# MrTornado24/FENeRF

Hardware: NVIDIA H100
Metric: rendered faces/sec at 128px x 24 samples/ray (higher is better)
Workload: dtype f16 operands / f32 accumulate (wgmma) + f32 refinement

## Files before the change

### fenerf_b200/csrc/layout.h

```cpp
#pragma once
#include <stddef.h>
#include <stdint.h>
#include "../../include/fenerf_b200.h"

#define FN_H 256
#define FN_MAX_HIDDEN 15
#define FN_KCHUNK 64
#define FN_IMG_BYTES (256 * FN_KCHUNK * 2)
#define FN_SLOT_POS 0
#define FN_SLOT_DIR 16
#define FN_SLOT_FEAT 32
#define FN_SPLIT_SCALES (FN_MAX_HIDDEN + 3)

#define FN_HEAD_IMG_BYTES(rows) ((size_t)(FN_H / FN_KCHUNK) * (rows) * FN_KCHUNK * 2)
constexpr int FN_FEAT = 64;
constexpr int FN_FEAT_SIGMA_ROW = 0;

struct FnHead {
    size_t w;
    size_t img;
    int32_t n_out, w_rows, img_rows;
};

struct FnLayout {
// ... 138 lines not shown
        L->head_img_s = take(FN_HEAD_IMG_BYTES(32));
        L->head_img_lo = take(FN_HEAD_IMG_BYTES(32));
        L->rgb_img_s = take(FN_HEAD_IMG_BYTES(8));
        L->rgb_img_lo = take(FN_HEAD_IMG_BYTES(8));
        L->split_scale = take(2 * FN_SPLIT_SCALES * 4);
    }
    L->total = off;
    return 0;
}

#if defined(__CUDACC__)
__host__ __device__
#endif
static inline uint32_t fn_sw128_offset(uint32_t row, uint32_t k) {
    return (row >> 3) * 1024u + (row & 7u) * 128u + ((((k >> 3) ^ (row & 7u)) & 7u) << 4) + (k & 7u) * 2u;
}

#if defined(__CUDACC__)
__host__ __device__
#endif
static inline uint32_t fn_hidden_img_offset(uint32_t n, uint32_t k) {
    return (n >> 7) * 65536u + (k / FN_KCHUNK) * 16384u + fn_sw128_offset(n & 127u, k % FN_KCHUNK);
}
```

### fenerf_b200/csrc/pack.cu

```cuda
#include "common.cuh"

namespace fn {

namespace {

__device__ __forceinline__ __half f16_hi(float w) { return __float2half_rn(w); }
__device__ __forceinline__ __half f16_lo(float w) { return __float2half_rn(w - __half2float(__float2half_rn(w))); }

__global__ void pack_first_kernel(const float* __restrict__ w, int g, const float* __restrict__ b,
                                  float* __restrict__ wt, float* __restrict__ bo, unsigned char* __restrict__ img,
                                  unsigned char* __restrict__ img_lo) {
    int n = blockIdx.x * blockDim.x + threadIdx.x;
    if (n >= FN_H) return;
    const int in_dim = g + 3;
    bo[n] = b[n];
    for (int k = 0; k < FN_KCHUNK; ++k) *reinterpret_cast<__half*>(img + fn_sw128_offset(n, k)) = __float2half_rn(0.f);
    for (int k = 0; k < 3; ++k) {
        float v = w[n * in_dim + g + k];
        wt[k * FN_H + n] = v;
        *reinterpret_cast<__half*>(img + fn_sw128_offset(n, FN_SLOT_POS + k)) = f16_hi(v);
        *reinterpret_cast<__half*>(img + fn_sw128_offset(n, FN_SLOT_POS + 3 + k)) = f16_hi(v);
        *reinterpret_cast<__half*>(img + fn_sw128_offset(n, FN_SLOT_POS + 6 + k)) = f16_lo(v);
    }
    if (img_lo)
        for (int k = 0; k < FN_KCHUNK; ++k) *reinterpret_cast<__half*>(img_lo + fn_sw128_offset(n, k)) = __float2half_rn(0.f);
    for (int c = 0; c < g; ++c) {
        const float v = w[n * in_dim + c];
        wt[(3 + c) * FN_H + n] = v;
        *reinterpret_cast<__half*>(img + fn_sw128_offset(n, FN_SLOT_FEAT + c)) = f16_hi(v);
        *reinterpret_cast<__half*>(img_lo + fn_sw128_offset(n, FN_SLOT_FEAT + c)) = f16_lo(v);
    }
}

__global__ void pack_hidden_kernel(const float* __restrict__ w, const float* __restrict__ b, int in_dim, int x_off,
                                   int kx, int kx_pad, float* __restrict__ wt, float* __restrict__ bo,
                                   unsigned char* __restrict__ img) {
    __shared__ float tile[32][33];
    int k0 = blockIdx.x * 32, n0 = blockIdx.y * 32;
    int k_total = FN_H + kx_pad;
    for (int i = threadIdx.y; i < 32; i += blockDim.y) {
        int n = n0 + i, k = k0 + threadIdx.x;
        float v = 0.f;
        if (k < FN_H) v = w[(size_t)n * in_dim + x_off + k];
        else if (k - FN_H < kx) v = w[(size_t)n * in_dim + (k - FN_H)];
        tile[i][threadIdx.x] = v;
    }
    __syncthreads();
    for (int i = threadIdx.y; i < 32; i += blockDim.y) {
        int k = k0 + i, n = n0 + threadIdx.x;
        if (k < k_total) wt[(size_t)k * FN_H + n] = tile[threadIdx.x][i];
    }
    for (int i = threadIdx.y; i < 32; i += blockDim.y) {
        int n = n0 + i, k = k0 + threadIdx.x;
        if (k < FN_H)
            *reinterpret_cast<__half*>(img + fn_hidden_img_offset(n, k)) = __float2half_rn(tile[i][threadIdx.x]);
    }
    if (blockIdx.x == 0 && threadIdx.y == 0) bo[n0 + threadIdx.x] = b[n0 + threadIdx.x];
}

__global__ void pack_color0_ximg_kernel(const float* __restrict__ w, int in_dim, int g, unsigned char* __restrict__ img) {
    int n = blockIdx.x * blockDim.x + threadIdx.x;
    if (n >= FN_H) return;
    for (int k = 0; k < FN_KCHUNK; ++k) *reinterpret_cast<__half*>(img + fn_sw128_offset(n, k)) = __float2half_rn(0.f);
    for (int k = 0; k < 3; ++k) {
        float v = w[(size_t)n * in_dim + k];
        *reinterpret_cast<__half*>(img + fn_sw128_offset(n, FN_SLOT_DIR + k)) = f16_hi(v);
        *reinterpret_cast<__half*>(img + fn_sw128_offset(n, FN_SLOT_DIR + 3 + k)) = f16_hi(v);
        *reinterpret_cast<__half*>(img + fn_sw128_offset(n, FN_SLOT_DIR + 6 + k)) = f16_lo(v);
    }
    for (int c = 0; c < g; ++c)
        *reinterpret_cast<__half*>(img + fn_sw128_offset(n, FN_SLOT_FEAT + c)) = __float2half_rn(w[(size_t)n * in_dim + 3 + c]);
}

__global__ void pack_wo_dir_color0_kernel(const float* __restrict__ w, int g, int kx_pad, const float* __restrict__ b,
                                          float* __restrict__ wt, float* __restrict__ bo, unsigned char* __restrict__ img,
                                          unsigned char* __restrict__ ximg) {
    const int n = blockIdx.x;
    const size_t in_dim = (size_t)g + FN_H;
    for (int k = threadIdx.x; k < FN_H + kx_pad; k += blockDim.x) {
        float v = 0.f;
        if (k < FN_H) {
            v = w[n * in_dim + g + k];
            *reinterpret_cast<__half*>(img + fn_hidden_img_offset(n, k)) = __float2half_rn(v);
        } else if (k - FN_H >= 3 && k - FN_H < 3 + g) {
            v = w[n * in_dim + (k - FN_H - 3)];
        }
        wt[(size_t)k * FN_H + n] = v;
    }
    for (int k = threadIdx.x; k < FN_KCHUNK; k += blockDim.x) {
        const int c = k - FN_SLOT_FEAT;
        const float v = c >= 0 && c < g ? w[n * in_dim + c] : 0.f;
        *reinterpret_cast<__half*>(ximg + fn_sw128_offset(n, k)) = __float2half_rn(v);
    }
    if (threadIdx.x == 0) bo[n] = b[n];
}

__global__ void label_step1_kernel(const float* __restrict__ w3, const float* __restrict__ b3,
                                   const float* __restrict__ w2, const float* __restrict__ b2,
                                   double* __restrict__ u ) {
    int i = blockIdx.x, j = threadIdx.x;
    if (!w2) {
        u[i * (FN_H + 1) + j] = (double)w3[i * FN_H + j];
        if (j == 0) u[i * (FN_H + 1) + FN_H] = (double)b3[i];
        return;
    }
    double acc = 0.0;
// ... 343 lines not shown
        FN_REQUIRE(w && b, "weight/bias of hidden layer %d missing", l);
        if (L.bridge && is_c0) {
            FN_REQUIRE(!L.bridge_res || (bridge->pre_w && bridge->pre_b), "color_layer_pre missing");
            pack_bridge_color0_kernel<<<1, 256, 0, st>>>(w, L.bridge_res ? 3 + FN_H : 6, b,
                                                         L.bridge_res ? bridge->pre_w : nullptr,
                                                         L.bridge_res ? bridge->pre_b : nullptr,
                                                         (float*)(packed + L.hid_w32[l]), (float*)(packed + L.hid_b[l]),
                                                         packed + L.color0_ximg);
            FN_LAUNCH_OK("pack_bridge_color0_kernel");
            continue;
        }
        if (L.wo_dir && is_c0) {
            pack_wo_dir_color0_kernel<<<FN_H, 256, 0, st>>>(w, L.grid_channels, L.kx_pad, b, (float*)(packed + L.hid_w32[l]),
                                                            (float*)(packed + L.hid_b[l]), packed + L.hid_img[l],
                                                            packed + L.color0_ximg);
            FN_LAUNCH_OK("pack_wo_dir_color0_kernel");
            continue;
        }
        int in_dim = is_c0 ? L.kx + FN_H : FN_H;
        int x_off = is_c0 ? L.kx : 0;
        int kx = is_c0 ? L.kx : 0, kx_pad = is_c0 ? L.kx_pad : 0;
        dim3 grid((FN_H + kx_pad + 31) / 32, FN_H / 32), block(32, 8);
        pack_hidden_kernel<<<grid, block, 0, st>>>(w, b, in_dim, x_off, kx, kx_pad, (float*)(packed + L.hid_w32[l]),
                                                   (float*)(packed + L.hid_b[l]), packed + L.hid_img[l]);
        FN_LAUNCH_OK("pack_hidden_kernel");
        if (is_c0) {
            pack_color0_ximg_kernel<<<1, 256, 0, st>>>(w, in_dim, L.kx - 3, packed + L.color0_ximg);
            FN_LAUNCH_OK("pack_color0_ximg_kernel");
        }
    }
    FN_REQUIRE((L.bridge_res || (p->sigma_w && p->sigma_b)) && p->rgb_w && p->rgb_b, "sigma/rgb head parameters missing");
    pack_linear_head_kernel<<<1, 256, 0, st>>>(p->rgb_w, p->rgb_b, L.rgb, packed);
    FN_LAUNCH_OK("pack_linear_head_kernel");
    if (L.label_film) {
        pack_linear_head_kernel<<<1, 256, 0, st>>>(p->label_w[2], p->label_b[2], L.label, packed);
        FN_LAUNCH_OK("pack_linear_head_kernel");
    } else if (L.trunk_labels > 0) {
        for (int i = 0; i < 3; i += 2) FN_REQUIRE(p->label_w[i] && p->label_b[i], "label layer %d missing", i);
        FN_REQUIRE((p->label_w[1] == nullptr) == (p->label_b[1] == nullptr), "label layer 1: weight and bias must both be given or both be NULL");
        double* u = reinterpret_cast<double*>(packed + L.label_scratch);
        label_step1_kernel<<<L.label_dim, FN_H, 0, st>>>(p->label_w[2], p->label_b[2], p->label_w[1], p->label_b[1], u);
        FN_LAUNCH_OK("label_step1_kernel");
        label_step2_kernel<<<L.label_dim, FN_H, 0, st>>>(u, p->label_w[0], p->label_b[0], L.label_dim,
                                                         (float*)(packed + L.label_w));
        FN_LAUNCH_OK("label_step2_kernel");
        label_step3_kernel<<<1, 256, 0, st>>>((float*)(packed + L.label_w), L.label_dim);
        FN_LAUNCH_OK("label_step3_kernel");
// ... 42 lines not shown
```

### fenerf_b200/csrc/siren_fast.cu

```cuda
#include "siren_fast.cuh"

namespace fn {

int siren_fast_label_launch(const void* args, int blocks, cudaStream_t st);
int siren_fast_hd_launch(const void* args, int blocks, bool label_film, cudaStream_t st);
int siren_fast_grid_launch(const void* args, int blocks, cudaStream_t st);
int siren_fast_bridge_launch(const void* args, int blocks, cudaStream_t st);
int siren_fast_debug_launch(const void* args, int blocks, bool label_film, bool feature_head, int variant, cudaStream_t st);

namespace {

std::atomic<int> g_variant{0};
unsigned long long* g_trace = nullptr;
int g_trace_ctas = 0;

bool build_loads(const FnLayout& L, FastArgs& A, bool sigma_only) {
    A.n_loads = 0;
    auto push = [&](size_t src, uint32_t bytes) {
        if (A.n_loads < MAX_LOADS) A.loads[A.n_loads] = Load{(uint32_t)src, bytes};
        ++A.n_loads;
    };
    push(L.first_img, 2 * CHUNK);
    if (L.grid_trunk) push(L.first_img_lo, 2 * CHUNK);
    for (int l = 0; l < L.n_hidden; ++l) {
        if (l == L.trunk_hidden) {
            push(L.head_img, 4 * HEAD_CHUNK);
            if (sigma_only) return A.n_loads <= MAX_LOADS;
        }
        if (L.bridge && l == L.color0) {
            push(L.color0_ximg, 2 * CHUNK);
            continue;
        }
        push(L.hid_img[l], 2 * CHUNK);
        push(L.hid_img[l] + 2 * CHUNK, 2 * CHUNK);
        if (l == L.label_layer) push(L.label.img, (uint32_t)FN_HEAD_IMG_BYTES(L.label.img_rows));
        if (l == L.color0) push(L.color0_ximg, 2 * CHUNK);
        push(L.hid_img[l] + 4 * CHUNK, 2 * CHUNK);
        push(L.hid_img[l] + 6 * CHUNK, 2 * CHUNK);
    }
    push(L.rgb.img, (uint32_t)FN_HEAD_IMG_BYTES(L.rgb.img_rows));
    return A.n_loads <= MAX_LOADS;
}

}

int siren_fast_debug_variant(int variant, unsigned long long* trace, int trace_ctas) {
    FN_REQUIRE(variant >= 0 && variant <= 3, "unknown point-network variant %d", variant);
    FN_REQUIRE(variant < 2 || (trace && trace_ctas >= 1), "a timeline variant needs its trace buffer");
    g_trace = trace;
    g_trace_ctas = trace_ctas;
    g_variant.store(variant);
    return 0;
}

int siren_points_fast(const FnLayout& L, const unsigned char* packed, const float* points, const float* dirs, const float* film,
                      int batch, long long ppb, int dir_group, int lock_dirs, float* out, int sigma_only, cudaStream_t st,
                      float* sigma_out) {
    static_assert(sizeof(FastArgs) <= 4000, "kernel parameter block too large");
    static_assert(SMEM_TOTAL <= 232448, "one CTA per SM: 227 KB of shared memory");
    static_assert(FN_HEAD_IMG_BYTES(FN_FEAT) == SLOT_BYTES, "a feature-head image is one ring slot");
    const bool trunk_only = L.feature_head && sigma_only;
// ... 41 lines not shown
```

### fenerf_b200/csrc/siren_fast.cuh

```cuda
#pragma once
#include "common.cuh"
#include "siren_common.cuh"
#include "sm90.cuh"

namespace fn {

namespace {

using namespace sm90;

constexpr int TILE = 64;
constexpr int NTHREADS = 384;
constexpr int PROD_WARP = 8;
constexpr int RING = 6;
constexpr uint32_t SLOT_BYTES = 32768;
constexpr int XSTRIDE = 72;
constexpr uint32_t SMEM_X = RING * SLOT_BYTES;
constexpr int FRING = 2;
constexpr uint32_t FILM_BYTES = 2 * FN_H * 4;
constexpr uint32_t SMEM_FILM = SMEM_X + 2 * TILE * XSTRIDE * 2;
constexpr uint32_t SMEM_BAR = SMEM_FILM + 2 * FRING * FILM_BYTES;
constexpr uint32_t SMEM_TOTAL = SMEM_BAR + 16 * RING + 16 + 16 * 2 * FRING;
constexpr uint32_t SMEM_XLO = SMEM_TOTAL;
constexpr int XLO_STRIDE = 32;
// ... 46 lines not shown
    uint32_t bytes;
};

template <int kMaxLoads>
struct FastArgsT {
    Load loads[kMaxLoads];
    int n_loads;
    FnLayout L;
    const unsigned char* packed;
    const float* points;
    const float* dirs;
    const float* film;
    float* out;
    float* sigma_out;
    long long ppb, tiles_per_batch, n_tiles;
    int dir_group, lock_dirs;
    int sigma_only;
    unsigned long long* trace;
    int trace_ctas;
};
using FastArgs = FastArgsT<MAX_LOADS>;
using SplitArgs = FastArgsT<MAX_LOADS_SPLIT>;

__device__ __forceinline__ void wg_bar(int wg) { asm volatile("bar.sync %0, 128;" ::"r"(1 + wg) : "memory"); }

template <bool kLabelFilm, bool kFeatureHead = false, int kSoftSin = kSoftSinEvery, bool kTrace = false,
          bool kGridTrunk = false, bool kBridge = false, bool kSplit = false>
__global__ void __launch_bounds__(NTHREADS, 1)
    siren_fast_kernel(const __grid_constant__ FastArgsT<kSplit ? MAX_LOADS_SPLIT : MAX_LOADS> a) {
    constexpr int RING = kSplit ? RING_SPLIT : fn::RING;
    constexpr uint32_t SMEM_X = kSplit ? SPLIT_SMEM_X : fn::SMEM_X;
    constexpr uint32_t SMEM_FILM = kSplit ? SPLIT_SMEM_FILM : fn::SMEM_FILM;
    constexpr uint32_t SMEM_BAR = kSplit ? SPLIT_SMEM_BAR : fn::SMEM_BAR;
    constexpr uint32_t SMEM_XLO = kSplit ? SPLIT_SMEM_XLO : fn::SMEM_XLO;
    extern __shared__ __align__(1024) unsigned char smem[];
    const uint32_t sbase = smem_u32(smem);
    const int warp = threadIdx.x >> 5, lane = threadIdx.x & 31;
    const uint32_t bar_full = sbase + SMEM_BAR, bar_empty = bar_full + 8 * RING, bar_turn = bar_empty + 8 * RING;
    const uint32_t bar_ffull = bar_turn + 16, bar_fempty = bar_ffull + 8 * 2 * FRING;
    unsigned long long* tbuf = nullptr;
    uint32_t tn = 0;
    if constexpr (kTrace)
        if (lane == 0 && (int)blockIdx.x < a.trace_ctas) tbuf = a.trace + ((size_t)blockIdx.x * TRACE_WARPS + warp) * TRACE_CAP;
    auto trace = [&](int kind, int group = 0) {
        if constexpr (kTrace)
            if (tbuf && tn < TRACE_CAP)
// ... 60 lines not shown
                }
            }
        }
        return;
    }

    asm volatile("setmaxnreg.inc.sync.aligned.u32 232;\n" ::: "memory");
    const int wg = warp >> 2, q = lane & 3;
    const int tid = threadIdx.x & 127;
    const int r0 = (warp & 3) * 16 + (lane >> 2);
    const FnLayout& L = a.L;
    const int C = L.out_dim;
    const float* sigma_w = reinterpret_cast<const float*>(a.packed + L.sigma_w);
    const float* label_w = reinterpret_cast<const float*>(a.packed + L.label_w);
    const int trunk_labels = (kLabelFilm || kFeatureHead) ? 0 : L.trunk_labels;
    const int sigma_row = kFeatureHead ? FN_FEAT_SIGMA_ROW : L.sigma_row;
    const int rgb_rows = kFeatureHead ? FN_FEAT : L.rgb.w_rows;
    const int label_rows = kFeatureHead ? FN_FEAT : L.label.w_rows;
    __half* xs = reinterpret_cast<__half*>(smem + SMEM_X) + wg * TILE * XSTRIDE;
    uint32_t it = 0;
    auto acquire = [&](uint32_t& slot) -> uint32_t {
        slot = it % RING;
        trace(TR_ACQ_WAIT);
        mbar_wait(bar_full + 8 * slot, (it / RING) & 1u);
        trace(TR_ACQ_DONE);
        ++it;
        return sbase + slot * SLOT_BYTES;
    };
    auto release = [&](uint32_t slot) {
        __syncwarp();
        if (lane == 0) mbar_arrive(bar_empty + 8 * slot);
    };
    uint32_t turns = 0;
    uint32_t fit = 0;
    auto film_acquire = [&]() -> const float4* {
        const uint32_t e = wg * FRING + fit % FRING;
        trace(TR_FILM_WAIT);
        mbar_wait(bar_ffull + 8 * e, (fit / FRING) & 1u);
        trace(TR_FILM_DONE);
        return reinterpret_cast<const float4*>(smem + SMEM_FILM + e * FILM_BYTES);
    };
    auto film_release = [&]() {
        const uint32_t e = wg * FRING + fit % FRING;
        ++fit;
        __syncwarp();
        if (lane == 0) mbar_arrive(bar_fempty + 8 * e);
    };
    auto turn_begin = [&]() {
        trace(TR_TURN_WAIT);
        mbar_wait(bar_turn + 8 * wg, (turns & 1u) ^ (wg == 0 ? 1u : 0u));
        trace(TR_TURN_DONE);
    };
    auto turn_end = [&](int group) {
        trace(TR_COMMIT, group);
        ++turns;
        __syncwarp();
        if (lane == 0) mbar_arrive(bar_turn + 8 * (wg ^ 1));
    };
    auto xfrag = [&](int s, uint32_t (&f)[4]) {
        const __half* p = xs + r0 * XSTRIDE + 16 * s + 2 * q;
        f[0] = *reinterpret_cast<const uint32_t*>(p);
        f[1] = *reinterpret_cast<const uint32_t*>(p + 8 * XSTRIDE);
        f[2] = *reinterpret_cast<const uint32_t*>(p + 8);
        f[3] = *reinterpret_cast<const uint32_t*>(p + 8 * XSTRIDE + 8);
    };

    for (long long pair = blockIdx.x; pair < n_pairs; pair += gridDim.x) {
        const long long tile = pair * 2 + wg;
        const bool tile_ok = tile < a.n_tiles;
        const long long b = tile_ok ? tile / a.tiles_per_batch : 0;
        const long long p0 = tile_ok ? (tile % a.tiles_per_batch) * TILE : a.ppb;
        trace(TR_PAIR);

// ... 31 lines not shown
                if (valid && (kGridTrunk || (L.grid_channels > 0 && !a.sigma_only))) {
                    float feat[32];
                    grid_features32(reinterpret_cast<const float*>(a.packed + L.grid), L.grid_res, pos[0], pos[1], pos[2], feat);
#pragma unroll
                    for (int i = 0; i < 32; ++i) split_f16(feat[i], slots[FN_SLOT_FEAT + i], lo[i]);
                }
                __half* xlo = reinterpret_cast<__half*>(smem + SMEM_XLO) + (wg * TILE + tid) * XLO_STRIDE;
#pragma unroll
                for (int i = 0; i < 4; ++i) reinterpret_cast<uint4*>(xlo)[i] = reinterpret_cast<const uint4*>(lo)[i];
            } else if (L.grid_channels > 0 && valid && !a.sigma_only) {
                float feat[32];
                grid_features32_h(reinterpret_cast<const __half*>(a.packed + L.grid16), L.grid_res, pos[0], pos[1], pos[2], feat);
#pragma unroll
                for (int i = 0; i < 32; ++i) slots[FN_SLOT_FEAT + i] = __float2half_rn(feat[i]);
            }
#pragma unroll
            for (int i = 0; i < 8; ++i)
                reinterpret_cast<uint4*>(xs + tid * XSTRIDE)[i] = reinterpret_cast<const uint4*>(slots)[i];
        }
        wg_bar(wg);

        uint32_t act[16][4];
        uint32_t nxt[8][4];
        float d[64];
        auto film_epi = [&](const float4* fs, int h, uint32_t (&dst)[8][4]) {
#pragma unroll
            for (int j = 0; j < 16; ++j) {
                const float4 e = fs[64 * h + 4 * j + q];
                const bool soft = kSoftSin > 0 && j % (kSoftSin > 0 ? kSoftSin : 1) == kSoftSin - 1;
                auto sn = [soft](float x) { return soft ? soft_sinf(x) : __sinf(x); };
                dst[j >> 1][(j & 1) * 2] = pack_half2(sn(fmaf(e.x, d[4 * j], e.z)), sn(fmaf(e.y, d[4 * j + 1], e.w)));
                dst[j >> 1][(j & 1) * 2 + 1] = pack_half2(sn(fmaf(e.x, d[4 * j + 2], e.z)), sn(fmaf(e.y, d[4 * j + 3], e.w)));
            }
            trace(TR_EPI_DONE);
        };
        auto act_hi = [&]() -> uint32_t (&)[8][4] { return *reinterpret_cast<uint32_t (*)[8][4]>(&act[8]); };
        auto film_epi_split = [&](const float4* fs, int h, uint32_t (&dst)[8][4], uint32_t (&lo)[8][4]) {
#pragma unroll
            for (int j = 0; j < 16; ++j) {
                const float4 e = fs[64 * h + 4 * j + q];
#pragma unroll
                for (int rr = 0; rr < 2; ++rr) {
                    const float s0 = soft_sinf(fmaf(e.x, d[4 * j + 2 * rr], e.z));
                    const float s1 = soft_sinf(fmaf(e.y, d[4 * j + 2 * rr + 1], e.w));
                    const __half2 hi = __floats2half2_rn(s0, s1);
                    const float2 hf = __half22float2(hi);
                    dst[j >> 1][(j & 1) * 2 + rr] = *reinterpret_cast<const uint32_t*>(&hi);
// ... 21 lines not shown
            wg_bar(wg);
        };
        uint32_t lo0[8][4], lo1[8][4];

        {
            uint32_t xf[4], slot, slot_lo = 0, w_lo = 0;
            uint32_t xg[2][4], xl[2][4];
            const float4* fs = nullptr;
            xfrag(0, xf);
            if constexpr (kGridTrunk) {
                const __half* xlo = reinterpret_cast<const __half*>(smem + SMEM_XLO) + wg * TILE * XLO_STRIDE;
#pragma unroll
                for (int s = 0; s < 2; ++s) {
                    xfrag(2 + s, xg[s]);
                    const __half* p = xlo + r0 * XLO_STRIDE + 16 * s + 2 * q;
                    xl[s][0] = *reinterpret_cast<const uint32_t*>(p);
                    xl[s][1] = *reinterpret_cast<const uint32_t*>(p + 8 * XLO_STRIDE);
                    xl[s][2] = *reinterpret_cast<const uint32_t*>(p + 8);
                    xl[s][3] = *reinterpret_cast<const uint32_t*>(p + 8 * XLO_STRIDE + 8);
                }
            }
            const uint32_t w = acquire(slot);
            if constexpr (kGridTrunk) w_lo = acquire(slot_lo);
#pragma unroll
            for (int h = 0; h < 2; ++h) {
                turn_begin();
                wg_fence();
                mma_rs_n128(d, xf, desc_kmajor(w + h * CHUNK), 0u);
                if constexpr (kGridTrunk)
#pragma unroll
                    for (int s = 0; s < 2; ++s) {
                        mma_rs_n128(d, xg[s], desc_kmajor(w + h * CHUNK + 32 * (2 + s)), 1u);
                        mma_rs_n128(d, xl[s], desc_kmajor(w + h * CHUNK + 32 * (2 + s)), 1u);
                        mma_rs_n128(d, xg[s], desc_kmajor(w_lo + h * CHUNK + 32 * (2 + s)), 1u);
                    }
                wg_commit();
                turn_end(TG_FIRST);
                wg_wait<0>();
                trace(TR_MMA_DONE);
                fence_regs(d);
                fence_regs(xf);
                if constexpr (kGridTrunk) { fence_regs(xg); fence_regs(xl); }
                if (h == 0) fs = film_acquire();
                if constexpr (kSplit) {
                    if (h == 0) film_epi_split(fs, 0, nxt, lo0);
                    else film_epi_split(fs, 1, act_hi(), lo1);
                } else {
                    if (h == 0) film_epi(fs, 0, nxt);
                    else film_epi(fs, 1, act_hi());
                }
            }
            release(slot);
            if constexpr (kGridTrunk) release(slot_lo);
            film_release();
            if constexpr (kSplit) alo_store(lo0, lo1);
#pragma unroll
            for (int s = 0; s < 8; ++s)
#pragma unroll
                for (int i = 0; i < 4; ++i) act[s][i] = nxt[s][i];
        }

        bool stop = false;
        for (int l = 0; l < L.n_hidden && !stop; ++l) {
            if (l == L.trunk_hidden) {
                float dh[16];
                uint32_t slot, slot_lo = 0, w_lo = 0;
                const uint32_t w = acquire(slot);
                if constexpr (kSplit) w_lo = acquire(slot_lo);
                turn_begin();
                wg_fence();
#pragma unroll
                for (int c = 0; c < 4; ++c)
#pragma unroll
                    for (int k = 0; k < 4; ++k) mma_rs_n32(dh, act[4 * c + k], desc_kmajor(w + c * HEAD_CHUNK + 32 * k), (c | k) ? 1u : 0u);
                if constexpr (kSplit)
#pragma unroll
                    for (int c = 0; c < 4; ++c)
#pragma unroll
                        for (int k = 0; k < 4; ++k) {
                            mma_ss_n32(dh, alo_desc(4 * c + k), desc_kmajor(w + c * HEAD_CHUNK + 32 * k), 1u);
                            mma_rs_n32(dh, act[4 * c + k], desc_kmajor(w_lo + c * HEAD_CHUNK + 32 * k), 1u);
                        }
// ... 64 lines not shown
                        }
                    }
                    if (!a.sigma_only) wg_bar(wg);
                }
                if (a.sigma_only) { stop = true; break; }
                if constexpr (kLabelFilm) {
                    constexpr int kLabN = kFeatureHead ? FN_FEAT : 32;
                    constexpr uint32_t kLabChunk = kFeatureHead ? FEAT_CHUNK : HEAD_CHUNK;
                    float dl[kLabN / 2];
                    uint32_t slot_h = 0, w_h = 0;
                    const float4* fs = nullptr;
#pragma unroll
                    for (int h = 0; h < 2; ++h) {
                        uint32_t sl[2];
                        turn_begin();
                        wg_fence();
#pragma unroll
                        for (int sb = 0; sb < 2; ++sb) {
                            const uint32_t w = acquire(sl[sb]);
#pragma unroll
                            for (int c = 0; c < 2; ++c)
#pragma unroll
                                for (int k = 0; k < 4; ++k)
                                    mma_rs_n128(d, act[8 * sb + 4 * c + k], desc_kmajor(w + c * CHUNK + 32 * k), (sb | c | k) ? 1u : 0u);
                        }
                        wg_commit();
                        turn_end(TG_LABEL_LAYER);
                        wg_wait<0>();
                        trace(TR_MMA_DONE);
                        fence_regs(d);
                        fence_regs(act);
                        release(sl[0]);
                        release(sl[1]);
                        if (h == 0) fs = film_acquire();
                        film_epi(fs, h, nxt);
                        if (h == 0) w_h = acquire(slot_h);
                        turn_begin();
                        wg_fence();
#pragma unroll
                        for (int s = 0; s < 8; ++s) {
                            const int g = 8 * h + s;
                            const uint64_t desc = desc_kmajor(w_h + (g >> 2) * kLabChunk + 32 * (g & 3));
                            if constexpr (kFeatureHead) mma_rs_n64(dl, nxt[s], desc, (h | s) ? 1u : 0u);
                            else mma_rs_n32(dl, nxt[s], desc, (h | s) ? 1u : 0u);
                        }
                        wg_commit();
                        turn_end(TG_LABEL_HEAD);
                        wg_wait<0>();
                        trace(TR_MMA_DONE);
                        fence_regs(dl);
                        fence_regs(nxt);
                    }
                    release(slot_h);
// ... 69 lines not shown
                                mma_rs_n128(d, xl[s], desc_kmajor(w_x + off), 1u);
                                mma_rs_n128(d, xf[1 + s], desc_kmajor(w_xl + off), 1u);
                            }
                        wg_commit();
                        turn_end(TG_COLOR0);
                        wg_wait<0>();
                        trace(TR_MMA_DONE);
                        fence_regs(d);
                        fence_regs(xf);
                        fence_regs(xl);
                        release(slot_x);
                        if (grid) release(slot_xl);
                    }
                    if (h == 0) fs = film_acquire();
                    if (h == 0) film_epi_split(fs, 0, nxt, lo0);
                    else film_epi_split(fs, 1, act_hi(), lo1);
                }
                film_release();
                alo_store(lo0, lo1);
#pragma unroll
                for (int s = 0; s < 8; ++s)
#pragma unroll
                    for (int i = 0; i < 4; ++i) act[s][i] = nxt[s][i];
                continue;
            }
            const bool narrow = kBridge && c0;
            const int nx = kBridge ? 2 : !kGridTrunk && L.grid_channels > 0 ? 3 : 1;
            uint32_t xf[3][4];
            if (c0)
#pragma unroll
                for (int s = 0; s < 3; ++s) xfrag(1 + s, xf[s]);
            uint32_t slot_x = 0, w_x = 0;
            const float4* fs = nullptr;
#pragma unroll
            for (int h = 0; h < 2; ++h) {
                uint32_t sl[2] = {0u, 0u};
                if (narrow && h == 0) w_x = acquire(slot_x);
                turn_begin();
                wg_fence();
                if (!narrow)
#pragma unroll
                    for (int sb = 0; sb < 2; ++sb) {
                        const uint32_t w = acquire(sl[sb]);
#pragma unroll
                        for (int c = 0; c < 2; ++c)
#pragma unroll
                            for (int k = 0; k < 4; ++k)
                                mma_rs_n128(d, act[8 * sb + 4 * c + k], desc_kmajor(w + c * CHUNK + 32 * k), (sb | c | k) ? 1u : 0u);
                    }
                if (c0) {
                    if (h == 0 && !narrow) w_x = acquire(slot_x);
#pragma unroll
                    for (int s = 0; s < 3; ++s)
                        if (s < nx) mma_rs_n128(d, xf[s], desc_kmajor(w_x + h * CHUNK + 32 * (1 + s)), (narrow && s == 0) ? 0u : 1u);
                }
                wg_commit();
                turn_end(c0 ? TG_COLOR0 : TG_HIDDEN);
                wg_wait<0>();
                trace(TR_MMA_DONE);
                fence_regs(d);
                fence_regs(act);
                fence_regs(xf);
                if (!narrow) {
                    release(sl[0]);
                    release(sl[1]);
                }
                if (c0 && h == 1) release(slot_x);
                if (h == 0) fs = film_acquire();
                if (h == 0) film_epi(fs, 0, nxt);
                else film_epi(fs, 1, act_hi());
            }
            film_release();
#pragma unroll
            for (int s = 0; s < 8; ++s)
#pragma unroll
                for (int i = 0; i < 4; ++i) act[s][i] = nxt[s][i];
        }
        if (stop) continue;

        if constexpr (kFeatureHead) {
            float dr[32];
            uint32_t slot;
            const uint32_t w = acquire(slot);
            turn_begin();
            wg_fence();
#pragma unroll
            for (int c = 0; c < 4; ++c)
#pragma unroll
                for (int k = 0; k < 4; ++k) mma_rs_n64(dr, act[4 * c + k], desc_kmajor(w + c * FEAT_CHUNK + 32 * k), (c | k) ? 1u : 0u);
            wg_commit();
            turn_end(TG_OUT_HEAD);
            wg_wait<0>();
            trace(TR_MMA_DONE);
            fence_regs(dr);
            fence_regs(act);
            release(slot);
            const float* rgb_b = reinterpret_cast<const float*>(a.packed + L.rgb.w) + rgb_rows * FN_H;
#pragma unroll
            for (int rr = 0; rr < 2; ++rr) {
// ... 69 lines not shown
```

### fenerf_b200/csrc/sm90.cuh

```cuda
#pragma once
#include "common.cuh"

namespace fn {
namespace sm90 {

__device__ __forceinline__ uint32_t smem_u32(const void* p) { return (uint32_t)__cvta_generic_to_shared(p); }

__device__ __forceinline__ void mbar_init(uint32_t bar, uint32_t count) {
    asm volatile("mbarrier.init.shared::cta.b64 [%0], %1;" ::"r"(bar), "r"(count));
}
__device__ __forceinline__ void fence_barrier_init() { asm volatile("fence.mbarrier_init.release.cluster;" ::: "memory"); }
__device__ __forceinline__ void mbar_arrive(uint32_t bar) {
    asm volatile("{\n\t.reg .b64 st;\n\tmbarrier.arrive.shared::cta.b64 st, [%0];\n\t}" ::"r"(bar) : "memory");
}
__device__ __forceinline__ void mbar_arrive_expect_tx(uint32_t bar, uint32_t bytes) {
    asm volatile("{\n\t.reg .b64 st;\n\tmbarrier.arrive.expect_tx.shared::cta.b64 st, [%0], %1;\n\t}" ::"r"(bar), "r"(bytes)
                 : "memory");
}
__device__ __forceinline__ void mbar_wait(uint32_t bar, uint32_t parity) {
    const long long t0 = clock64();
    for (;;) {
        uint32_t done;
        asm volatile("{\n\t.reg .pred p;\n\tmbarrier.try_wait.parity.shared::cta.b64 p, [%1], %2;\n\tselp.u32 %0, 1, 0, p;\n\t}"
                     : "=r"(done) : "r"(bar), "r"(parity) : "memory");
// ... 33 lines not shown
}
template <int M, int N>
__device__ __forceinline__ void fence_regs(uint32_t (&r)[M][N]) {
#pragma unroll
    for (int i = 0; i < M; ++i) fence_regs(r[i]);
}

__device__ __forceinline__ uint64_t desc_sw128(uint32_t smem_addr, uint32_t lbo, uint32_t sbo) {
    return (uint64_t)((smem_addr >> 4) & 0x3FFF) | ((uint64_t)((lbo >> 4) & 0x3FFF) << 16) |
           ((uint64_t)((sbo >> 4) & 0x3FFF) << 32) | (1ull << 62);
}
__device__ __forceinline__ uint64_t desc_kmajor(uint32_t smem_addr) { return desc_sw128(smem_addr, 16, 1024); }

__device__ __forceinline__ uint32_t pack_half2(float a, float b) {
    __half2 h = __floats2half2_rn(a, b);
    return *reinterpret_cast<uint32_t*>(&h);
}
__device__ __forceinline__ void split_f16(float v, __half& hi, __half& lo) {
    hi = __float2half_rn(v);
    lo = __float2half_rn(v - __half2float(hi));
}


__device__ __forceinline__ void mma_rs_n128(float (&d)[64], const uint32_t (&a)[4], uint64_t b_desc, uint32_t acc) {
    asm volatile(
        "{\n\t.reg .pred p;\n\tsetp.ne.b32 p, %69, 0;\n\t"
        "wgmma.mma_async.sync.aligned.m64n128k16.f32.f16.f16 {%0, %1, %2, %3, %4, %5, %6, %7, %8, %9, %10, %11, %12, %13, %14, %15, %16, %17, %18, %19, %20, %21, %22, %23, %24, %25, %26, %27, %28, %29, %30, %31, %32, %33, %34, %35, %36, %37, %38, %39, %40, %41, %42, %43, %44, %45, %46, %47, %48, %49, %50, %51, %52, %53, %54, %55, %56, %57, %58, %59, %60, %61, %62, %63}, {%64, %65, %66, %67}, %68, p, 1, 1, 0;\n\t}"
        : "+f"(d[0]), "+f"(d[1]), "+f"(d[2]), "+f"(d[3]), "+f"(d[4]), "+f"(d[5]), "+f"(d[6]), "+f"(d[7]), "+f"(d[8]), "+f"(d[9]), "+f"(d[10]), "+f"(d[11]), "+f"(d[12]), "+f"(d[13]), "+f"(d[14]), "+f"(d[15]), "+f"(d[16]), "+f"(d[17]), "+f"(d[18]), "+f"(d[19]), "+f"(d[20]), "+f"(d[21]), "+f"(d[22]), "+f"(d[23]), "+f"(d[24]), "+f"(d[25]), "+f"(d[26]), "+f"(d[27]), "+f"(d[28]), "+f"(d[29]), "+f"(d[30]), "+f"(d[31]), "+f"(d[32]), "+f"(d[33]), "+f"(d[34]), "+f"(d[35]), "+f"(d[36]), "+f"(d[37]), "+f"(d[38]), "+f"(d[39]), "+f"(d[40]), "+f"(d[41]), "+f"(d[42]), "+f"(d[43]), "+f"(d[44]), "+f"(d[45]), "+f"(d[46]), "+f"(d[47]), "+f"(d[48]), "+f"(d[49]), "+f"(d[50]), "+f"(d[51]), "+f"(d[52]), "+f"(d[53]), "+f"(d[54]), "+f"(d[55]), "+f"(d[56]), "+f"(d[57]), "+f"(d[58]), "+f"(d[59]), "+f"(d[60]), "+f"(d[61]), "+f"(d[62]), "+f"(d[63])
        : "r"(a[0]), "r"(a[1]), "r"(a[2]), "r"(a[3]), "l"(b_desc), "r"(acc));
}

__device__ __forceinline__ void mma_rs_n32(float (&d)[16], const uint32_t (&a)[4], uint64_t b_desc, uint32_t acc) {
    asm volatile(
        "{\n\t.reg .pred p;\n\tsetp.ne.b32 p, %21, 0;\n\t"
        "wgmma.mma_async.sync.aligned.m64n32k16.f32.f16.f16 {%0, %1, %2, %3, %4, %5, %6, %7, %8, %9, %10, %11, %12, %13, %14, %15}, {%16, %17, %18, %19}, %20, p, 1, 1, 0;\n\t}"
        : "+f"(d[0]), "+f"(d[1]), "+f"(d[2]), "+f"(d[3]), "+f"(d[4]), "+f"(d[5]), "+f"(d[6]), "+f"(d[7]), "+f"(d[8]), "+f"(d[9]), "+f"(d[10]), "+f"(d[11]), "+f"(d[12]), "+f"(d[13]), "+f"(d[14]), "+f"(d[15])
        : "r"(a[0]), "r"(a[1]), "r"(a[2]), "r"(a[3]), "l"(b_desc), "r"(acc));
}

__device__ __forceinline__ void mma_rs_n64(float (&d)[32], const uint32_t (&a)[4], uint64_t b_desc, uint32_t acc) {
    asm volatile(
        "{\n\t.reg .pred p;\n\tsetp.ne.b32 p, %37, 0;\n\t"
        "wgmma.mma_async.sync.aligned.m64n64k16.f32.f16.f16 {%0, %1, %2, %3, %4, %5, %6, %7, %8, %9, %10, %11, %12, %13, %14, %15, %16, %17, %18, %19, %20, %21, %22, %23, %24, %25, %26, %27, %28, %29, %30, %31}, {%32, %33, %34, %35}, %36, p, 1, 1, 0;\n\t}"
        : "+f"(d[0]), "+f"(d[1]), "+f"(d[2]), "+f"(d[3]), "+f"(d[4]), "+f"(d[5]), "+f"(d[6]), "+f"(d[7]), "+f"(d[8]), "+f"(d[9]), "+f"(d[10]), "+f"(d[11]), "+f"(d[12]), "+f"(d[13]), "+f"(d[14]), "+f"(d[15]), "+f"(d[16]), "+f"(d[17]), "+f"(d[18]), "+f"(d[19]), "+f"(d[20]), "+f"(d[21]), "+f"(d[22]), "+f"(d[23]), "+f"(d[24]), "+f"(d[25]), "+f"(d[26]), "+f"(d[27]), "+f"(d[28]), "+f"(d[29]), "+f"(d[30]), "+f"(d[31])
        : "r"(a[0]), "r"(a[1]), "r"(a[2]), "r"(a[3]), "l"(b_desc), "r"(acc));
}
// ... 43 lines not shown
```

Baseline: 601.2.

## Use full-width m64n256 wgmma for hidden layers with K-chunk-major weight images

Hidden and first layers now issue m64n256k16 wgmma over all 256 outputs at once, instead of two n128 halves that each re-stream the activation fragments. Weight images for non-label layers are repacked K-chunk-major so each ring slot holds one 64-wide K chunk for all outputs, and slots are released as per-chunk commit groups retire. The FiLM epilogue runs once over the full 128-register accumulator, and mbarrier waits now vote across the warp. The cost is that accumulator registers double, which raises register pressure and risks spills or lower occupancy.

Result: no change. 608.4, median of 6 (+1.2%).

```diff
diff --git a/fenerf_b200/csrc/layout.h b/fenerf_b200/csrc/layout.h
--- a/fenerf_b200/csrc/layout.h
+++ b/fenerf_b200/csrc/layout.h
@@ -184,3 +184,10 @@
 static inline uint32_t fn_hidden_img_offset(uint32_t n, uint32_t k) {
     return (n >> 7) * 65536u + (k / FN_KCHUNK) * 16384u + fn_sw128_offset(n & 127u, k % FN_KCHUNK);
 }
+
+#if defined(__CUDACC__)
+__host__ __device__
+#endif
+static inline uint32_t fn_hidden_img_chunk_offset(uint32_t n, uint32_t k) {
+    return (k / FN_KCHUNK) * (uint32_t)FN_IMG_BYTES + fn_sw128_offset(n, k % FN_KCHUNK);
+}
diff --git a/fenerf_b200/csrc/pack.cu b/fenerf_b200/csrc/pack.cu
--- a/fenerf_b200/csrc/pack.cu
+++ b/fenerf_b200/csrc/pack.cu
@@ -34,7 +34,7 @@
 
 __global__ void pack_hidden_kernel(const float* __restrict__ w, const float* __restrict__ b, int in_dim, int x_off,
                                    int kx, int kx_pad, float* __restrict__ wt, float* __restrict__ bo,
-                                   unsigned char* __restrict__ img) {
+                                   unsigned char* __restrict__ img, int half_major) {
     __shared__ float tile[32][33];
     int k0 = blockIdx.x * 32, n0 = blockIdx.y * 32;
     int k_total = FN_H + kx_pad;
@@ -53,7 +53,8 @@
     for (int i = threadIdx.y; i < 32; i += blockDim.y) {
         int n = n0 + i, k = k0 + threadIdx.x;
         if (k < FN_H)
-            *reinterpret_cast<__half*>(img + fn_hidden_img_offset(n, k)) = __float2half_rn(tile[i][threadIdx.x]);
+            *reinterpret_cast<__half*>(img + (half_major ? fn_hidden_img_offset(n, k) : fn_hidden_img_chunk_offset(n, k))) =
+                __float2half_rn(tile[i][threadIdx.x]);
     }
     if (blockIdx.x == 0 && threadIdx.y == 0) bo[n0 + threadIdx.x] = b[n0 + threadIdx.x];
 }
@@ -81,7 +82,7 @@
         float v = 0.f;
         if (k < FN_H) {
             v = w[n * in_dim + g + k];
-            *reinterpret_cast<__half*>(img + fn_hidden_img_offset(n, k)) = __float2half_rn(v);
+            *reinterpret_cast<__half*>(img + fn_hidden_img_chunk_offset(n, k)) = __float2half_rn(v);
         } else if (k - FN_H >= 3 && k - FN_H < 3 + g) {
             v = w[n * in_dim + (k - FN_H - 3)];
         }
@@ -471,7 +472,7 @@
         int kx = is_c0 ? L.kx : 0, kx_pad = is_c0 ? L.kx_pad : 0;
         dim3 grid((FN_H + kx_pad + 31) / 32, FN_H / 32), block(32, 8);
         pack_hidden_kernel<<<grid, block, 0, st>>>(w, b, in_dim, x_off, kx, kx_pad, (float*)(packed + L.hid_w32[l]),
-                                                   (float*)(packed + L.hid_b[l]), packed + L.hid_img[l]);
+                                                   (float*)(packed + L.hid_b[l]), packed + L.hid_img[l], is_label ? 1 : 0);
         FN_LAUNCH_OK("pack_hidden_kernel");
         if (is_c0) {
             pack_color0_ximg_kernel<<<1, 256, 0, st>>>(w, in_dim, L.kx - 3, packed + L.color0_ximg);
diff --git a/fenerf_b200/csrc/siren_fast.cu b/fenerf_b200/csrc/siren_fast.cu
--- a/fenerf_b200/csrc/siren_fast.cu
+++ b/fenerf_b200/csrc/siren_fast.cu
@@ -31,12 +31,16 @@
             push(L.color0_ximg, 2 * CHUNK);
             continue;
         }
-        push(L.hid_img[l], 2 * CHUNK);
-        push(L.hid_img[l] + 2 * CHUNK, 2 * CHUNK);
-        if (l == L.label_layer) push(L.label.img, (uint32_t)FN_HEAD_IMG_BYTES(L.label.img_rows));
+        if (l == L.label_layer) {
+            push(L.hid_img[l], 2 * CHUNK);
+            push(L.hid_img[l] + 2 * CHUNK, 2 * CHUNK);
+            push(L.label.img, (uint32_t)FN_HEAD_IMG_BYTES(L.label.img_rows));
+            push(L.hid_img[l] + 4 * CHUNK, 2 * CHUNK);
+            push(L.hid_img[l] + 6 * CHUNK, 2 * CHUNK);
+            continue;
+        }
+        for (int c = 0; c < FN_H / FN_KCHUNK; ++c) push(L.hid_img[l] + c * SLOT_BYTES, SLOT_BYTES);
         if (l == L.color0) push(L.color0_ximg, 2 * CHUNK);
-        push(L.hid_img[l] + 4 * CHUNK, 2 * CHUNK);
-        push(L.hid_img[l] + 6 * CHUNK, 2 * CHUNK);
     }
     push(L.rgb.img, (uint32_t)FN_HEAD_IMG_BYTES(L.rgb.img_rows));
     return A.n_loads <= MAX_LOADS;
diff --git a/fenerf_b200/csrc/siren_fast.cuh b/fenerf_b200/csrc/siren_fast.cuh
--- a/fenerf_b200/csrc/siren_fast.cuh
+++ b/fenerf_b200/csrc/siren_fast.cuh
@@ -92,6 +92,17 @@
 using FastArgs = FastArgsT<MAX_LOADS>;
 using SplitArgs = FastArgsT<MAX_LOADS_SPLIT>;
 
+__device__ __forceinline__ void mbar_wait_warp(uint32_t bar, uint32_t parity) {
+    const long long t0 = clock64();
+    for (;;) {
+        uint32_t done;
+        asm volatile("{\n\t.reg .pred p;\n\tmbarrier.try_wait.parity.shared::cta.b64 p, [%1], %2;\n\tselp.u32 %0, 1, 0, p;\n\t}"
+                     : "=r"(done) : "r"(bar), "r"(parity) : "memory");
+        if (__all_sync(0xffffffffu, done)) return;
+        if (clock64() - t0 > 100000000000LL) __trap();
+    }
+}
+
 __device__ __forceinline__ void wg_bar(int wg) { asm volatile("bar.sync %0, 128;" ::"r"(1 + wg) : "memory"); }
 
 template <bool kLabelFilm, bool kFeatureHead = false, int kSoftSin = kSoftSinEvery, bool kTrace = false,
@@ -198,7 +209,7 @@
     auto acquire = [&](uint32_t& slot) -> uint32_t {
         slot = it % RING;
         trace(TR_ACQ_WAIT);
-        mbar_wait(bar_full + 8 * slot, (it / RING) & 1u);
+        mbar_wait_warp(bar_full + 8 * slot, (it / RING) & 1u);
         trace(TR_ACQ_DONE);
         ++it;
         return sbase + slot * SLOT_BYTES;
@@ -212,7 +223,7 @@
     auto film_acquire = [&]() -> const float4* {
         const uint32_t e = wg * FRING + fit % FRING;
         trace(TR_FILM_WAIT);
-        mbar_wait(bar_ffull + 8 * e, (fit / FRING) & 1u);
+        mbar_wait_warp(bar_ffull + 8 * e, (fit / FRING) & 1u);
         trace(TR_FILM_DONE);
         return reinterpret_cast<const float4*>(smem + SMEM_FILM + e * FILM_BYTES);
     };
@@ -224,7 +235,7 @@
     };
     auto turn_begin = [&]() {
         trace(TR_TURN_WAIT);
-        mbar_wait(bar_turn + 8 * wg, (turns & 1u) ^ (wg == 0 ? 1u : 0u));
+        mbar_wait_warp(bar_turn + 8 * wg, (turns & 1u) ^ (wg == 0 ? 1u : 0u));
         trace(TR_TURN_DONE);
     };
     auto turn_end = [&](int group) {
@@ -302,7 +313,20 @@
 
         uint32_t act[16][4];
         uint32_t nxt[8][4];
-        float d[64];
+        constexpr int kAcc = kSplit ? 64 : 128;
+        float d[kAcc];
+        auto d_half = [&]() -> float (&)[64] { return *reinterpret_cast<float (*)[64]>(&d[0]); };
+        auto film_epi_layer = [&](const float4* fs) {
+#pragma unroll
+            for (int j = 0; j < kAcc / 4; ++j) {
+                const float4 e = fs[4 * j + q];
+                const bool soft = kSoftSin > 0 && (j % 16) % (kSoftSin > 0 ? kSoftSin : 1) == kSoftSin - 1;
+                auto sn = [soft](float x) { return soft ? soft_sinf(x) : __sinf(x); };
+                act[j >> 1][(j & 1) * 2] = pack_half2(sn(fmaf(e.x, d[4 * j], e.z)), sn(fmaf(e.y, d[4 * j + 1], e.w)));
+                act[j >> 1][(j & 1) * 2 + 1] = pack_half2(sn(fmaf(e.x, d[4 * j + 2], e.z)), sn(fmaf(e.y, d[4 * j + 3], e.w)));
+            }
+            trace(TR_EPI_DONE);
+        };
         auto film_epi = [&](const float4* fs, int h, uint32_t (&dst)[8][4]) {
 #pragma unroll
             for (int j = 0; j < 16; ++j) {
@@ -370,17 +394,39 @@
             }
             const uint32_t w = acquire(slot);
             if constexpr (kGridTrunk) w_lo = acquire(slot_lo);
-#pragma unroll
-            for (int h = 0; h < 2; ++h) {
+            if constexpr (kSplit) {
+#pragma unroll
+                for (int h = 0; h < 2; ++h) {
+                    turn_begin();
+                    wg_fence();
+                    mma_rs_n128(d, xf, desc_kmajor(w + h * CHUNK), 0u);
+                    wg_commit();
+                    turn_end(TG_FIRST);
+                    wg_wait<0>();
+                    trace(TR_MMA_DONE);
+                    fence_regs(d);
+                    fence_regs(xf);
+                    if (h == 0) fs = film_acquire();
+                    if (h == 0) film_epi_split(fs, 0, nxt, lo0);
+                    else film_epi_split(fs, 1, act_hi(), lo1);
+                }
+                release(slot);
+                film_release();
+                alo_store(lo0, lo1);
+#pragma unroll
+                for (int s = 0; s < 8; ++s)
+#pragma unroll
+                    for (int i = 0; i < 4; ++i) act[s][i] = nxt[s][i];
+            } else {
                 turn_begin();
                 wg_fence();
-                mma_rs_n128(d, xf, desc_kmajor(w + h * CHUNK), 0u);
+                mma_rs_n256(d, xf, desc_kmajor(w), 0u);
                 if constexpr (kGridTrunk)
 #pragma unroll
                     for (int s = 0; s < 2; ++s) {
-                        mma_rs_n128(d, xg[s], desc_kmajor(w + h * CHUNK + 32 * (2 + s)), 1u);
-                        mma_rs_n128(d, xl[s], desc_kmajor(w + h * CHUNK + 32 * (2 + s)), 1u);
-                        mma_rs_n128(d, xg[s], desc_kmajor(w_lo + h * CHUNK + 32 * (2 + s)), 1u);
+                        mma_rs_n256(d, xg[s], desc_kmajor(w + 32 * (2 + s)), 1u);
+                        mma_rs_n256(d, xl[s], desc_kmajor(w + 32 * (2 + s)), 1u);
+                        mma_rs_n256(d, xg[s], desc_kmajor(w_lo + 32 * (2 + s)), 1u);
                     }
                 wg_commit();
                 turn_end(TG_FIRST);
@@ -389,23 +435,12 @@
                 fence_regs(d);
                 fence_regs(xf);
                 if constexpr (kGridTrunk) { fence_regs(xg); fence_regs(xl); }
-                if (h == 0) fs = film_acquire();
-                if constexpr (kSplit) {
-                    if (h == 0) film_epi_split(fs, 0, nxt, lo0);
-                    else film_epi_split(fs, 1, act_hi(), lo1);
-                } else {
-                    if (h == 0) film_epi(fs, 0, nxt);
-                    else film_epi(fs, 1, act_hi());
-                }
-            }
-            release(slot);
-            if constexpr (kGridTrunk) release(slot_lo);
-            film_release();
-            if constexpr (kSplit) alo_store(lo0, lo1);
-#pragma unroll
-            for (int s = 0; s < 8; ++s)
-#pragma unroll
-                for (int i = 0; i < 4; ++i) act[s][i] = nxt[s][i];
+                release(slot);
+                if constexpr (kGridTrunk) release(slot_lo);
+                fs = film_acquire();
+                film_epi_layer(fs);
+                film_release();
+            }
         }
 
         bool stop = false;
@@ -516,13 +551,14 @@
                             for (int c = 0; c < 2; ++c)
 #pragma unroll
                                 for (int k = 0; k < 4; ++k)
-                                    mma_rs_n128(d, act[8 * sb + 4 * c + k], desc_kmajor(w + c * CHUNK + 32 * k), (sb | c | k) ? 1u : 0u);
+                                    mma_rs_n128(d_half(), act[8 * sb + 4 * c + k], desc_kmajor(w + c * CHUNK + 32 * k),
+                                                (sb | c | k) ? 1u : 0u);
                         }
                         wg_commit();
                         turn_end(TG_LABEL_LAYER);
                         wg_wait<0>();
                         trace(TR_MMA_DONE);
-                        fence_regs(d);
+                        fence_regs(d_half());
                         fence_regs(act);
                         release(sl[0]);
                         release(sl[1]);
@@ -638,59 +674,64 @@
                 for (int s = 0; s < 8; ++s)
 #pragma unroll
                     for (int i = 0; i < 4; ++i) act[s][i] = nxt[s][i];
-                continue;
-            }
-            const bool narrow = kBridge && c0;
-            const int nx = kBridge ? 2 : !kGridTrunk && L.grid_channels > 0 ? 3 : 1;
-            uint32_t xf[3][4];
-            if (c0)
-#pragma unroll
-                for (int s = 0; s < 3; ++s) xfrag(1 + s, xf[s]);
-            uint32_t slot_x = 0, w_x = 0;
-            const float4* fs = nullptr;
-#pragma unroll
-            for (int h = 0; h < 2; ++h) {
-                uint32_t sl[2] = {0u, 0u};
-                if (narrow && h == 0) w_x = acquire(slot_x);
-                turn_begin();
-                wg_fence();
-                if (!narrow)
-#pragma unroll
-                    for (int sb = 0; sb < 2; ++sb) {
-                        const uint32_t w = acquire(sl[sb]);
-#pragma unroll
-                        for (int c = 0; c < 2; ++c)
-#pragma unroll
-                            for (int k = 0; k < 4; ++k)
-                                mma_rs_n128(d, act[8 * sb + 4 * c + k], desc_kmajor(w + c * CHUNK + 32 * k), (sb | c | k) ? 1u : 0u);
-                    }
-                if (c0) {
-                    if (h == 0 && !narrow) w_x = acquire(slot_x);
-#pragma unroll
-                    for (int s = 0; s < 3; ++s)
-                        if (s < nx) mma_rs_n128(d, xf[s], desc_kmajor(w_x + h * CHUNK + 32 * (1 + s)), (narrow && s == 0) ? 0u : 1u);
-                }
-                wg_commit();
-                turn_end(c0 ? TG_COLOR0 : TG_HIDDEN);
-                wg_wait<0>();
-                trace(TR_MMA_DONE);
-                fence_regs(d);
-                fence_regs(act);
-                fence_regs(xf);
-                if (!narrow) {
+            } else {
+                const bool narrow = kBridge && c0;
+                const int nx = kBridge ? 2 : !kGridTrunk && L.grid_channels > 0 ? 3 : 1;
+                uint32_t xf[3][4];
+                if (c0)
+#pragma unroll
+                    for (int s = 0; s < 3; ++s) xfrag(1 + s, xf[s]);
+                if (narrow) {
+                    uint32_t slot_x;
+                    const uint32_t w_x = acquire(slot_x);
+                    turn_begin();
+                    wg_fence();
+                    mma_rs_n256(d, xf[0], desc_kmajor(w_x + 32), 0u);
+                    mma_rs_n256(d, xf[1], desc_kmajor(w_x + 64), 1u);
+                    wg_commit();
+                    turn_end(TG_COLOR0);
+                    wg_wait<0>();
+                    trace(TR_MMA_DONE);
+                    fence_regs(d);
+                    fence_regs(xf);
+                    release(slot_x);
+                } else {
+                    uint32_t sl[4], slot_x = 0;
+                    turn_begin();
+                    wg_fence();
+#pragma unroll
+                    for (int c = 0; c < 4; ++c) {
+                        const uint32_t w = acquire(sl[c]);
+#pragma unroll
+                        for (int k = 0; k < 4; ++k) {
+                            mma_rs_n256(d, act[4 * c + k], desc_kmajor(w + 32 * k), (c | k) ? 1u : 0u);
+                        }
+                        if (c == 3 && c0) {
+                            const uint32_t w_x = acquire(slot_x);
+#pragma unroll
+                            for (int s = 0; s < 3; ++s)
+                                if (s < nx) mma_rs_n256(d, xf[s], desc_kmajor(w_x + 32 * (1 + s)), 1u);
+                        }
+                        wg_commit();
+                    }
+                    turn_end(c0 ? TG_COLOR0 : TG_HIDDEN);
+                    wg_wait<3>();
                     release(sl[0]);
+                    wg_wait<2>();
                     release(sl[1]);
-                }
-                if (c0 && h == 1) release(slot_x);
-                if (h == 0) fs = film_acquire();
-                if (h == 0) film_epi(fs, 0, nxt);
-                else film_epi(fs, 1, act_hi());
-            }
-            film_release();
-#pragma unroll
-            for (int s = 0; s < 8; ++s)
-#pragma unroll
-                for (int i = 0; i < 4; ++i) act[s][i] = nxt[s][i];
+                    wg_wait<1>();
+                    release(sl[2]);
+                    wg_wait<0>();
+                    trace(TR_MMA_DONE);
+                    fence_regs(d);
+                    fence_regs(act);
+                    fence_regs(xf);
+                    release(sl[3]);
+                    if (c0) release(slot_x);
+                }
+                film_epi_layer(film_acquire());
+                film_release();
+            }
         }
         if (stop) continue;
 
diff --git a/fenerf_b200/csrc/sm90.cuh b/fenerf_b200/csrc/sm90.cuh
--- a/fenerf_b200/csrc/sm90.cuh
+++ b/fenerf_b200/csrc/sm90.cuh
@@ -79,6 +79,14 @@
 }
 
 
+__device__ __forceinline__ void mma_rs_n256(float (&d)[128], const uint32_t (&a)[4], uint64_t b_desc, uint32_t acc) {
+    asm volatile(
+        "{\n\t.reg .pred p;\n\tsetp.ne.b32 p, %133, 0;\n\t"
+        "wgmma.mma_async.sync.aligned.m64n256k16.f32.f16.f16 {%0, %1, %2, %3, %4, %5, %6, %7, %8, %9, %10, %11, %12, %13, %14, %15, %16, %17, %18, %19, %20, %21, %22, %23, %24, %25, %26, %27, %28, %29, %30, %31, %32, %33, %34, %35, %36, %37, %38, %39, %40, %41, %42, %43, %44, %45, %46, %47, %48, %49, %50, %51, %52, %53, %54, %55, %56, %57, %58, %59, %60, %61, %62, %63, %64, %65, %66, %67, %68, %69, %70, %71, %72, %73, %74, %75, %76, %77, %78, %79, %80, %81, %82, %83, %84, %85, %86, %87, %88, %89, %90, %91, %92, %93, %94, %95, %96, %97, %98, %99, %100, %101, %102, %103, %104, %105, %106, %107, %108, %109, %110, %111, %112, %113, %114, %115, %116, %117, %118, %119, %120, %121, %122, %123, %124, %125, %126, %127}, {%128, %129, %130, %131}, %132, p, 1, 1, 0;\n\t}"
+        : "+f"(d[0]), "+f"(d[1]), "+f"(d[2]), "+f"(d[3]), "+f"(d[4]), "+f"(d[5]), "+f"(d[6]), "+f"(d[7]), "+f"(d[8]), "+f"(d[9]), "+f"(d[10]), "+f"(d[11]), "+f"(d[12]), "+f"(d[13]), "+f"(d[14]), "+f"(d[15]), "+f"(d[16]), "+f"(d[17]), "+f"(d[18]), "+f"(d[19]), "+f"(d[20]), "+f"(d[21]), "+f"(d[22]), "+f"(d[23]), "+f"(d[24]), "+f"(d[25]), "+f"(d[26]), "+f"(d[27]), "+f"(d[28]), "+f"(d[29]), "+f"(d[30]), "+f"(d[31]), "+f"(d[32]), "+f"(d[33]), "+f"(d[34]), "+f"(d[35]), "+f"(d[36]), "+f"(d[37]), "+f"(d[38]), "+f"(d[39]), "+f"(d[40]), "+f"(d[41]), "+f"(d[42]), "+f"(d[43]), "+f"(d[44]), "+f"(d[45]), "+f"(d[46]), "+f"(d[47]), "+f"(d[48]), "+f"(d[49]), "+f"(d[50]), "+f"(d[51]), "+f"(d[52]), "+f"(d[53]), "+f"(d[54]), "+f"(d[55]), "+f"(d[56]), "+f"(d[57]), "+f"(d[58]), "+f"(d[59]), "+f"(d[60]), "+f"(d[61]), "+f"(d[62]), "+f"(d[63]), "+f"(d[64]), "+f"(d[65]), "+f"(d[66]), "+f"(d[67]), "+f"(d[68]), "+f"(d[69]), "+f"(d[70]), "+f"(d[71]), "+f"(d[72]), "+f"(d[73]), "+f"(d[74]), "+f"(d[75]), "+f"(d[76]), "+f"(d[77]), "+f"(d[78]), "+f"(d[79]), "+f"(d[80]), "+f"(d[81]), "+f"(d[82]), "+f"(d[83]), "+f"(d[84]), "+f"(d[85]), "+f"(d[86]), "+f"(d[87]), "+f"(d[88]), "+f"(d[89]), "+f"(d[90]), "+f"(d[91]), "+f"(d[92]), "+f"(d[93]), "+f"(d[94]), "+f"(d[95]), "+f"(d[96]), "+f"(d[97]), "+f"(d[98]), "+f"(d[99]), "+f"(d[100]), "+f"(d[101]), "+f"(d[102]), "+f"(d[103]), "+f"(d[104]), "+f"(d[105]), "+f"(d[106]), "+f"(d[107]), "+f"(d[108]), "+f"(d[109]), "+f"(d[110]), "+f"(d[111]), "+f"(d[112]), "+f"(d[113]), "+f"(d[114]), "+f"(d[115]), "+f"(d[116]), "+f"(d[117]), "+f"(d[118]), "+f"(d[119]), "+f"(d[120]), "+f"(d[121]), "+f"(d[122]), "+f"(d[123]), "+f"(d[124]), "+f"(d[125]), "+f"(d[126]), "+f"(d[127])
+        : "r"(a[0]), "r"(a[1]), "r"(a[2]), "r"(a[3]), "l"(b_desc), "r"(acc));
+}
+
 __device__ __forceinline__ void mma_rs_n128(float (&d)[64], const uint32_t (&a)[4], uint64_t b_desc, uint32_t acc) {
     asm volatile(
         "{\n\t.reg .pred p;\n\tsetp.ne.b32 p, %69, 0;\n\t"
```
